# xudoong/EdgeVisionTransformer

Measured on AMD Instinct MI355X. Metric: images/sec DeiT-base/16-224 bs=512 @1/2/4/8 GPU; % bf16 MFMA roofline, higher is better.
Workload: dtype bf16; 1 GPU; deit_base/16-224 forward, bs=512 per GPU, bf16; model=deit_base, global_batch=512, per_gpu_batch=512, seq_len=197, parallelism=dp1, gemm_variant=automatic, lanes=1

## Files before the change

edgevisiontransformer_amd/csrc/attention.hip:

```cpp
#include "common.h"
#include "evt_internal.h"

namespace evt {

namespace {

template <int NKT>
__device__ __forceinline__ float prescale_nonpositive(f32x4 (&s)[NKT], float scale_log2) {
  if (scale_log2 > 0.f) return scale_log2;
#pragma unroll
  for (int kt = 0; kt < NKT; ++kt) s[kt] = s[kt] * scale_log2;
  return 1.f;
}


template <int NKT, bool PLAIN_STORE>
__device__ __forceinline__ void attn_tile_bf16(const AttnParams& p, const EVT_LDS char* Ks,
                                               const EVT_LDS char* Vs, u32x4 qf0, u32x4 qf1,
                                               int qt, int b, int h, int lane) {
  constexpr int ROWB = 128;
  const int g = lane >> 4, c16 = lane & 15, sw = lane & 7;
  f32x4 s[NKT];
#pragma unroll
  for (int kt = 0; kt < NKT; ++kt) {
// ... 155 lines not shown
  }
}

template <int NKT, int WAVES, int NQW, bool NT = false, bool NTQ = NT, bool Q0 = false>
__device__ __forceinline__ void attn_stage_bf16(const AttnParams& p, EVT_LDS char* Ks,
                                                EVT_LDS char* Vs, u32x4 (&qf)[NQW][2], int b,
                                                int h, int wave, int lane) {
  constexpr int NP = NKT * 16, ROWB = 128;
  const bf16* qkv = (const bf16*)p.qkv + b * p.sb + h * p.sh;
  const int g = lane >> 4, c16 = lane & 15;
#pragma unroll
  for (int i = 0; i < NQW; ++i) {
    if (Q0 && wave != 0) break;
    const int qi = min((wave + WAVES * i) * 16 + c16, p.N - 1);
    const bf16* qrow = qkv + (int64_t)qi * p.ldq;
    if (NTQ) {
      qf[i][0] = __builtin_nontemporal_load((const u32x4*)(qrow + 8 * g));
      qf[i][1] = __builtin_nontemporal_load((const u32x4*)(qrow + 8 * (g + 4)));
    } else {
      qf[i][0] = *(const u32x4*)(qrow + 8 * g);
      qf[i][1] = *(const u32x4*)(qrow + 8 * (g + 4));
    }
  }
  const int srow = lane >> 3, sslot = lane & 7;
  for (int i = wave; i < NP / 8; i += WAVES) {
    const int row = i * 8 + srow;
    const int gr = min(row, p.N - 1);
    const bf16* rp = qkv + (int64_t)gr * p.ldq + ((sslot ^ srow) * 8);
    if (NT) {
      __builtin_amdgcn_global_load_lds(rp + p.ko, Ks + i * 8 * ROWB, 16, 0, 2);
// ... 805 lines not shown
  (void)hipFuncSetAttribute((const void*)attn_f32_kernel<14>, hipFuncAttributeMaxDynamicSharedMemorySize,
                      2 * 14 * 16 * 256);
  (void)hipFuncSetAttribute((const void*)attn_f32_kernel<16>, hipFuncAttributeMaxDynamicSharedMemorySize,
                      2 * 16 * 16 * 256);
}

}

bool attention_cls_ok(int dtype, const AttnParams& p) {
  return dtype == DT_BF16 && p.hd == 64 && p.N <= 256 && !p.q8;
}

hipError_t attention_launch(int dtype, const AttnParams& p_in, hipStream_t s) {
  if (p_in.B <= 0) return hipSuccess;
  if (p_in.cls_only && !attention_cls_ok(dtype, p_in)) return hipErrorInvalidValue;
  if (p_in.N <= 0 || p_in.N > EVT_ATTN_MAX_TOKENS || p_in.H <= 0 || p_in.hd <= 0 || p_in.hd > 128)
    return hipErrorInvalidValue;
  if (p_in.N > 256 && p_in.q8) return hipErrorInvalidValue;
  if (p_in.N > 256 && !(p_in.scale_log2 > 0.f && p_in.scale_log2 < INFINITY)) return hipErrorInvalidValue;
  AttnParams p = p_in;
  const bool strided = p.sb || p.sh || p.ko || p.vo;
  if (strided) {
    if (dtype != DT_BF16 || p.hd != 64 || p.q8 || p.sb % 8 || p.sh % 8 || p.ldq % 8 || p.ko % 8 ||
        p.vo % 8 || p.ldq < 64 || p.ko < 0 || p.vo < 0 || p.sb < 0 || p.sh < 0)
      return hipErrorInvalidValue;
  } else {
    p.sb = (int64_t)p.N * p.ldq;
    p.sh = 64;
    p.ko = p.H * 64;
    p.vo = 2 * p.H * 64;
// ... 17 lines not shown
```

edgevisiontransformer_amd/csrc/encoder.cpp:

```cpp
#include "model.h"

using namespace evt;

namespace evt {

int build_encoder(evt_model* m, const float* const* w, hipStream_t s) {
  const int D = m->D;
  const int depth = (int)m->heads.size();
  const int qb = m->standard ? 1 : 0;
  m->layers.resize(depth);
  int k = 0;
  for (int i = 0; i < depth; ++i) {
    Layer& L = m->layers[i];
    L.heads = m->heads[i];
    L.hd = m->head_dim[i];
    L.inner = L.heads * L.hd;
    L.ffn = m->ffn[i];
    L.ffn_st = (int)round_up(L.ffn, PAD_N);
    EVT_RC(copy_vec(m, &L.ln1_g, w[k + 0], D, s));
    EVT_RC(copy_vec(m, &L.ln1_b, w[k + 1], D, s));
    if (m->mx8) {
      EVT_RC(copy_vec(m, &L.ln2_g, w[k + 5], D, s));
      EVT_RC(copy_vec(m, &L.ln2_b, w[k + 6], D, s));
      EVT_RC(make_mx8(m, &L.mqkv, w[k + 2], nullptr, D, 3 * L.inner, s));
// ... 19 lines not shown
void encoder_ws(const Shape& sh, int dtype, bool mx8, int B, size_t hbuf_bytes, WsLayout* l) {
  const size_t es = elem_size(dtype);
  if (dtype == DT_BF16)
    l->bufs.push_back({EVT_WS(sk), gemm_sk_bytes(), 4096, "memset stream-K flags"});
  const size_t rows = (size_t)B * sh.T;
  const size_t xb = (rows * sh.D + PAD_K) * es, ob = (rows * sh.max_inner + PAD_K) * es;
  const size_t stats_bytes = rows * stats_slots(sh.D) * 2 * sizeof(float);
  l->bufs.push_back({EVT_WS(x), xb, xb, "memset x"});
  l->bufs.push_back({EVT_WS(xm), xb, xb, "memset xm"});
  l->bufs.push_back({EVT_WS(sx), stats_bytes});
  l->bufs.push_back({EVT_WS(sm), stats_bytes});
  l->bufs.push_back({EVT_WS(qkv), rows * 3 * sh.max_inner * es});
  l->bufs.push_back({EVT_WS(o), ob, ob, "memset o"});
  l->bufs.push_back({EVT_WS(hbuf), hbuf_bytes});
  l->hbuf_bytes = hbuf_bytes;
  if (!mx8) l->bufs.push_back({EVT_WS(hc), (size_t)B * sh.max_ffn_st * es});
}

int dense_head(const evt_model* m, const DenseW& w, const DenseCall& c, hipStream_t s) {
  const int tiles = ((c.M + GEMM_BM - 1) / GEMM_BM) * (w.npad / GEMM_BN);
  int S = 1;
  while (S < 8 && tiles * S * 2 <= device_cus() && w.kpad % (S * 2 * PAD_K) == 0) S *= 2;
  const size_t part = (size_t)S * std::max(c.M, m->max_batch) * w.npad * sizeof(float);
  if (S < 2 || !m->ws.hbuf || part > m->ws.hbuf_bytes ||
      (c.flags & ~(EPI_BIAS | EPI_GELU | EPI_OUT_F32)))
    return dense(m, w, c, s);
  dense_work(m, w, c);
  const GemmParams p = gemm_operands(c.A, c.lda, w.w, w.kpad, w.npad, c.C, c.ldc, c.M, c.N, w.b,
                                     nullptr, 0, nullptr, 0, 0);
  EVT_HIP(gemm_splitk_launch(m->dtype, c.flags, p, S, (float*)m->ws.hbuf, s), "dense (split-K)");
  return EVT_OK;
}

int run_encoder(evt_model* m, ForwardCall& call) {
  const int B = call.B, D = m->D, T = m->sh.T, rows = B * T;
  hipStream_t s = call.s;
  const float log2e = 1.4426950408889634f;
  m->hm_layers = 0;
  m->tail_mode = 0;
  int block = 0;
  for (const Layer& L : m->layers) {
    const float scale_log2 = log2e / std::sqrt((float)L.hd);
    bool hm = false;
    {
      ProfScope ps(m, EVT_PROF_QKV, s);
      DenseCall c;
      c.flags = EPI_LNIN | EPI_BIAS;
      c.A = m->ws.x; c.lda = D; c.C = m->ws.qkv; c.ldc = 3 * L.inner; c.M = rows; c.N = 3 * L.inner;
      c.stats_in = m->ws.sx;
      if (L.hd == 64 && m->headmajor) {
        DenseCall h = c;
        h.flags |= EPI_HM;
        h.ldc = 64;
        h.P = T;
        if (gemm_headmajor_ok(m->dtype, h.flags, dense_params(m, L.qkv, h))) {
          c = h;
          hm = true;
          ++m->hm_layers;
        }
      }
      EVT_RC(dense(m, L.qkv, c, s));
    }
    AttnParams ap{m->ws.qkv, 3 * L.inner, m->ws.o, L.inner, T, L.heads, B, scale_log2};
    ap.hd = L.hd;
    if (hm) {
      ap.ldq = 64;
      ap.sb = (int64_t)L.heads * 3 * T * 64;
      ap.sh = (int64_t)3 * T * 64;
      ap.ko = T * 64;
      ap.vo = 2 * T * 64;
    }
    const bool last = block + 1 == (int)m->layers.size();
    bool full = !last;
    if (last && call.feat) {
      const evt_features_args* a = call.feat;
      full = a->tokens || (a->n_taps > 0 && a->tap_blocks[a->n_taps - 1] == block);
    }
    if (last) m->tail_mode = full ? 3 : 1;
    {
      ProfScope ps(m, EVT_PROF_ATTENTION, s);
      prof_work(m, 4.0 * B * L.heads * (double)T * T * L.hd,
                (double)rows * 4 * L.inner * elem_size(m->dtype));
      AttnParams aq = ap;
      aq.cls_only = !full && attention_cls_ok(m->dtype, ap);
      EVT_HIP(attention_launch(m->dtype, aq, s), "attention");
    }
    EVT_RC(attn_map(m, call, block, ap));
    EVT_RC(head_stats(m, call, block, ap));
    DenseCall co;
    co.flags = m->standard ? (EPI_BIAS | EPI_RESID | EPI_STATS)
                           : (EPI_BIAS | EPI_RESID | EPI_RESLN | EPI_STATS);
    co.A = m->ws.o; co.lda = L.inner; co.C = m->ws.xm; co.ldc = D; co.M = rows; co.N = D;
    co.resid = m->ws.x; co.ldr = D; co.rstats = m->ws.sx; co.rgamma = L.ln1_g; co.rbeta = L.ln1_b;
    co.stats_out = m->ws.sm;
    DenseCall c1;
    c1.flags = EPI_LNIN | EPI_BIAS | (m->standard ? EPI_GELU_ERF : EPI_GELU);
    c1.A = m->ws.xm; c1.lda = D; c1.C = m->ws.hbuf; c1.ldc = L.ffn_st; c1.M = rows; c1.N = L.ffn_st;
    c1.stats_in = m->ws.sm;
    DenseCall c2;
// ... 79 lines not shown
```

edgevisiontransformer_amd/csrc/evt_internal.h:

```cpp
#pragma once
#include <hip/hip_runtime.h>
#include <stddef.h>
#include <stdint.h>

namespace evt {

enum Dtype : int { DT_F32 = 0, DT_BF16 = 1 };

struct ImgAffine {
  float scale[4], shift[4];
};

enum : int {
  EPI_BIAS = 1,
  EPI_GELU = 2,
  EPI_RESID = 4,
  EPI_POS = 8,
  EPI_OUT_F32 = 16,
  EPI_LNIN = 32,
  EPI_RESLN = 64,
  EPI_STATS = 128,
  EPI_GELU_ERF = 256,
  EPI_OUT_MX8 = 512,
  EPI_GATHER = 1024,
// ... 22 lines not shown
  float eps;
  int nslots;
  int stats_step;
  int rs_step;
  int force_nt;
  int gR, gC;
  float g_inv_rr, g_inv_r;
  int gmode, gOW;
  const void* gzero;
  int* sk_flags;
  float* sk_part;
  int ks_chunk;
  int64_t ks_stride;
  int xgroups;
  int no_balance;
};
constexpr int GEMM_BM = 128;
constexpr int GEMM_BN = 128;
constexpr int PACK_N = 256;
constexpr int PAD_K = 64;
constexpr int PAD_N = 64;

hipError_t gemm_launch(int dtype, int flags, const GemmParams& p, hipStream_t s);
int device_cus();
bool gemm_headmajor_ok(int dtype, int flags, const GemmParams& p);
hipError_t gemm_splitk_launch(int dtype, int flags, const GemmParams& p, int S, float* part,
                              hipStream_t s);
void gemm_set_variant(int v);
size_t gemm_sk_bytes();
void gemm_sk_bind(void* ws, GemmParams& p);
hipError_t pack_weight(int dtype, const float* W, const float* row_scale, int K, int N, void* Wp,
                       int Kpad, int Npad, hipStream_t s);
hipError_t to_bf16_launch(const float* x, void* y, int64_t n, hipStream_t s);
hipError_t ln_fold(int dtype, const void* Wp, int Kpad, const float* W, const float* beta,
                   const float* bias, int K, int N, float* colsum, float* cvec, int Npad,
                   hipStream_t s);

constexpr int EVT_ATTN_MAX_TOKENS = 4096;

struct AttnParams {
  const void* qkv; int64_t ldq;
  void* out;       int64_t ldo;
  int N;
  int H;
  int B;
  float scale_log2;
  uint8_t* q8 = nullptr;
  uint32_t* s8 = nullptr;
  int64_t ldq8 = 0;
  int rows8 = 0;
  int hd = 64;
  int64_t sb = 0, sh = 0;
  int ko = 0, vo = 0;
  int cls_only = 0;
};
hipError_t attention_launch(int dtype, const AttnParams& p, hipStream_t s);
bool attention_cls_ok(int dtype, const AttnParams& p);
hipError_t attn_probs_launch(int dtype, const AttnParams& p, int nq, float* out, hipStream_t s);
hipError_t head_stats_launch(int dtype, const AttnParams& p, int prefix, int grid_w, float* out,
                             hipStream_t s);


hipError_t layernorm_launch(int dtype, const float* x, int64_t ldx, void* y, int64_t ldy,
                            const float* gamma, const float* beta, int rows, int D, float eps,
                            hipStream_t s);

hipError_t export_rows_launch(int dtype, const void* x, int64_t ldx, int64_t row_step, float* out,
                              const float* gamma, const float* beta, int rows, int D, float eps,
                              hipStream_t s);
// ... 121 lines not shown
  ImgAffine aff{};
  const void* w;
  int64_t ldw;
  const float* bias;
  const float* gamma;
  const float* beta;
  void* x;
  float* stats;
  int B, S, nslots;
  float eps;
};
hipError_t swin_embed96_launch(const SwinEmbedParams& p, hipStream_t s);
int gemm_variant();
inline bool gemm_auto() {
  const int v = gemm_variant();
  return v == 0 || v == 30 || v == 31;
}
bool gemm_variant_supported(int v);

struct Mx8GemmParams {
  const uint8_t* A;  int64_t lda;
  const uint32_t* As; int64_t ldas;
  const uint8_t* W;  int64_t ldw;
  const uint32_t* Ws; int64_t ldws;
  void* C;           int64_t ldc;
  uint32_t* Cs;      int64_t ldcs;
  int M, N, K;
  const float* bias;
  const void* resid; int64_t ldr;
  const float* rstats;
  const float* rgamma;
// ... 27 lines not shown
```

edgevisiontransformer_amd/csrc/gemm.hip:

```cpp
#include <type_traits>

#include "common.h"
#include "evt_internal.h"
#include "gemm_epi.h"
#include "gemm_nt.h"
#include "gemm_big8.h"
#include "gemm_big.h"
#include "gemm_pers.h"
#include "gemm_p384.h"
#include "gemm_sk.h"

namespace evt {

namespace {

enum : int {
  V_AUTO = 0,
  V_NT = 1,
  V_BIG_PLAIN = 2,
  V_BIG_SCHED = 6,
  V_BIG8 = 8,
  V_PERS = 9,
  V_STREAMK = 16,
  V_P384 = 30,
  V_NO_P384 = 31,
  V_NO_BALANCE = 36,
};
thread_local int g_gemm_variant = V_AUTO;

int g_num_cus = 0;
const int g_grid_balance = [] {
  const char* e = std::getenv("EVT_GRID_BALANCE");
  return (e && e[0] >= '0' && e[0] <= '2') ? e[0] - '0' : 1;
}();

int num_cus() {
  if (!g_num_cus) {
    int dev = 0;
    hipGetDevice(&dev);
    hipDeviceGetAttribute(&g_num_cus, hipDeviceAttributeMultiprocessorCount, dev);
  }
  return g_num_cus;
// ... 20 lines not shown
         fl == (EPI_BIAS | EPI_RESID | EPI_RESLN | EPI_STATS);
}

constexpr bool p384_fl(int fl) {
  return fl == (EPI_BIAS | EPI_RESID | EPI_RESLN | EPI_STATS) ||
         fl == (EPI_BIAS | EPI_RESID | EPI_STATS) || fl == (EPI_LNIN | EPI_BIAS | EPI_GELU) ||
         fl == (EPI_LNIN | EPI_BIAS);
}

bool use_big(const GemmParams& p, int flags) {
  if (p.force_nt || p.rs_step > 1) return false;
  if ((p.ntiles * GEMM_BN) % BIG_BN) return false;
  if (std::max(std::max(p.lda, p.ldw), std::max(p.ldc, p.resid ? p.ldr : (int64_t)0)) > BIG_MAX_LD)
    return false;
  if (!(flags & EPI_OUT_F32) && p.vec_ok < 2) return false;
  const int v = (g_gemm_variant == V_NO_P384 || g_gemm_variant == V_NO_BALANCE) ? V_AUTO
                                                                                : g_gemm_variant;
  if (v == V_NT) return false;
  if (v != V_AUTO) return true;
  const int64_t G = num_cus();
  const int64_t t256 = (int64_t)((p.M + 255) / 256) * (p.ntiles * GEMM_BN / 256);
  const int64_t t128 = (int64_t)((p.M + 127) / 128) * p.ntiles;
  return (t256 + G - 1) / G <= 0.5 * (double)((t128 + G - 1) / G);
}

bool pers_wide(const GemmParams& p, int flags) {
  return (flags & (EPI_LNIN | EPI_RESLN)) && p.nslots > 8;
}

bool use_pers(const GemmParams& p, int flags) {
  const int v = g_gemm_variant;
  if (v != V_AUTO && v != V_PERS && v != V_STREAMK && v != V_NO_P384 && v != V_NO_BALANCE)
    return false;
  if (p.N % 8 || p.vec_ok < 2 || p.force_nt || p.rs_step > 1) return false;
  if ((flags & (EPI_LNIN | EPI_RESLN)) && (p.nslots > 12 || p.nslots % 2 || p.stats_step > 1))
    return false;
  if (pers_wide(p, flags) &&
      (!pers_wide_fl(flags) || p.K / 64 < PERS_WIDE_MIN_NK || v == V_STREAMK))
    return false;
  if ((flags & EPI_POS) && (!p.resid || p.ldr % 8 || p.P <= 0 || p.M >= (1 << 22))) return false;
  return true;
}

int pers_xgroups(int ntiles, int G, int total) {
  if (G != 256 || total <= G) return 1;
  return (ntiles % 2 == 0 && ntiles / 2 >= 3) ? 2 : 1;
}

bool use_p384(const GemmParams& p, int flags) {
  const int v = g_gemm_variant;
  if ((v != V_AUTO && v != V_P384) || p.N % 384 || p.vec_ok < 2 || p.K < 64) return false;
  if (p.force_nt || p.rs_step > 1) return false;
  if (std::max(std::max(p.lda, p.ldw), std::max(p.ldc, p.resid ? p.ldr : (int64_t)0)) > BIG_MAX_LD)
    return false;
  if ((flags & (EPI_LNIN | EPI_RESLN)) && (p.nslots > 8 || p.nslots % 2 || p.stats_step > 1))
    return false;
  if ((flags & EPI_STATS) && 3 * (p.N / 384) > p.nslots) return false;
  return v == V_P384;
}

constexpr int SK_MAX_G = 256;

int sk_grid() { return min(num_cus(), SK_MAX_G) & ~7; }

bool use_sk(const GemmParams& p) {
  if (!p.sk_flags || !p.sk_part || g_gemm_variant != V_STREAMK) return false;
// ... 17 lines not shown
  if (g_gemm_variant == V_BIG_PLAIN)
    hipLaunchKernelGGL((gemm_big_kernel<FL, 0>), grid, dim3(512), 0, s, q);
  else if (g_gemm_variant == V_BIG8)
    hipLaunchKernelGGL((gemm_big_kernel<FL, 8>), grid, dim3(512), 0, s, q);
  else if constexpr ((FL & EPI_POS) != 0)
    hipLaunchKernelGGL((gemm_big_kernel<FL, 8>), grid, dim3(512), 0, s, q);
  else
    hipLaunchKernelGGL((gemm_big_kernel<FL, 6>), grid, dim3(512), 0, s, q);
  return hipGetLastError();
}

template <int FL>
hipError_t launch_pers(const GemmParams& p, hipStream_t s) {
  num_cus();
  GemmParams q = p;
  q.ntiles = (p.ntiles * GEMM_BN) / BIG_BN;
  const int total = ((p.M + BIG_BM - 1) / BIG_BM) * q.ntiles;
  int G = min(total, g_num_cus);
  if (G >= 8 && total > G) G &= ~7;
  const int rounds = (total + G - 1) / G;
  const int bal = (g_gemm_variant == V_NO_BALANCE || p.no_balance) ? 0 : g_grid_balance;
  if (total > G && G >= 8 && (bal == 2 || (bal == 1 && rounds <= 4)))
    G = min(G, (((total + rounds - 1) / rounds) + 7) & ~7);
  else if (total <= G && (G & 7) && ((G + 7) & ~7) <= max(g_num_cus, 8)) G = (G + 7) & ~7;
  q.xgroups = pers_xgroups(q.ntiles, G, total);
  if constexpr (pers_wide_fl(FL)) {
    if (pers_wide(p, FL)) {
      if (p.N % BIG_BN == 0)
        hipLaunchKernelGGL((gemm_pers_kernel<FL, false, true>), dim3(G), dim3(512), 0, s, q, total);
      else
        hipLaunchKernelGGL((gemm_pers_kernel<FL, true, true>), dim3(G), dim3(512), 0, s, q, total);
// ... 16 lines not shown
  if (G >= 8 && total > G) G &= ~7;
  hipLaunchKernelGGL((gemm_p384_kernel<FL>), dim3(G), dim3(512), 0, s, q, total);
  return hipGetLastError();
}

template <int FL>
hipError_t launch_sk(const GemmParams& p, hipStream_t s) {
  GemmParams q = p;
  q.ntiles = (p.ntiles * GEMM_BN) / BIG_BN;
  const int total = ((p.M + BIG_BM - 1) / BIG_BM) * q.ntiles;
  hipLaunchKernelGGL((gemm_sk_kernel<FL>), dim3(sk_grid()), dim3(512), 0, s, q, total);
  return hipGetLastError();
}

template <typename T, int FL>
hipError_t launch_t(const GemmParams& p, hipStream_t s) {
  if constexpr ((FL & EPI_HM) != 0) {
    if constexpr (std::is_same<T, bf16>::value && pers_fl(FL)) {
      if (headmajor_fits(p) && use_big(p, FL) && use_pers(p, FL)) return launch_pers<FL>(p, s);
    }
    return hipErrorNotSupported;
  } else if constexpr ((FL & (EPI_GATHER | EPI_SPLIT)) != 0) {
    if constexpr (std::is_same<T, bf16>::value) {
      constexpr bool MERGE = (FL & EPI_GATHER) != 0;
      const bool merge = MERGE && p.gmode == 1 && p.gR % 2 == 0 && p.gOW == p.gR / 2 &&
                         p.gC % 8 == 0 && p.K == 4 * p.gC;
      const bool unfold = !MERGE && p.gmode == 2 && p.gC == 64 && p.K == 9 * 64 && p.gzero &&
                          p.gOW == (p.gR + 1) / 2;
      if ((merge || unfold) && p.gR > 0 && p.M < (1 << 22) && use_big(p, FL) && use_pers(p, FL) &&
          !use_sk(p))
        return launch_pers<FL>(p, s);
    }
    return hipErrorNotSupported;
  } else {
    if constexpr (std::is_same<T, bf16>::value) {
      if constexpr (p384_fl(FL)) {
        if (use_p384(p, FL)) return launch_p384<FL>(p, s);
      }
      if (use_big(p, FL)) {
        if constexpr (pers_fl(FL)) {
          if (use_pers(p, FL)) return use_sk(p) ? launch_sk<FL>(p, s) : launch_pers<FL>(p, s);
        }
        return launch_big<FL>(p, s);
      }
    }
    const int mtiles = (p.M + GEMM_BM - 1) / GEMM_BM;
    hipLaunchKernelGGL((gemm_nt_kernel<T, FL>), dim3(mtiles * p.ntiles), dim3(256), 0, s, p);
    return hipGetLastError();
  }
// ... 110 lines not shown
  }
  s = wave_sum(s);
  c = wave_sum(c);
  if (lane == 0) {
    colsum[n] = s;
    cvec[n] = (n < N) ? c + (bias ? bias[n] : 0.f) : 0.f;
  }
}

}

int device_cus() { return num_cus(); }
void gemm_set_variant(int v) { g_gemm_variant = v; }
bool gemm_variant_supported(int v) {
  return v == V_AUTO || v == V_NT || v == V_BIG_PLAIN || v == V_BIG_SCHED || v == V_BIG8 ||
         v == V_PERS || v == V_STREAMK || v == V_P384 || v == V_NO_P384 || v == V_NO_BALANCE;
}
int gemm_variant() { return g_gemm_variant; }

size_t gemm_sk_bytes() { return 4096 + (size_t)SK_MAX_G * SK_SLOT_FLOATS * sizeof(float); }

void gemm_sk_bind(void* ws, GemmParams& p) {
  p.sk_flags = ws ? (int*)ws : nullptr;
  p.sk_part = ws ? (float*)((char*)ws + 4096) : nullptr;
}

bool gemm_headmajor_ok(int dtype, int flags, const GemmParams& p) {
  constexpr int F = EPI_LNIN | EPI_BIAS | EPI_HM;
  return dtype == DT_BF16 && (flags | EPI_HM) == F && p.K % PAD_K == 0 && p.K > 0 &&
         p.ntiles * GEMM_BN >= p.N && headmajor_fits(p) && use_big(p, F) && use_pers(p, F);
}

hipError_t gemm_launch(int dtype, int flags, const GemmParams& p, hipStream_t s) {
  if (p.M <= 0 || p.N <= 0) return hipSuccess;
  if (p.K % PAD_K != 0 || p.K <= 0) return hipErrorInvalidValue;
  if (p.ntiles * GEMM_BN < p.N) return hipErrorInvalidValue;
  return dtype == DT_BF16 ? dispatch<bf16>(flags, p, s) : dispatch<float>(flags, p, s);
}

hipError_t gemm_splitk_launch(int dtype, int flags, const GemmParams& p, int S, float* part,
                              hipStream_t s) {
  if (p.M <= 0 || p.N <= 0) return hipSuccess;
  if (S < 1 || p.K % (S * PAD_K) || (flags & ~(EPI_BIAS | EPI_GELU | EPI_OUT_F32)) || !part)
    return hipErrorInvalidValue;
  return dtype == DT_BF16 ? splitk_t<bf16>(flags, p, S, part, s) : splitk_t<float>(flags, p, S, part, s);
}

namespace {
__global__ void to_bf16_kernel(const float* __restrict__ x, bf16* __restrict__ y, int64_t n) {
  const int64_t i = (int64_t)blockIdx.x * blockDim.x + threadIdx.x;
  if (i < n) y[i] = (bf16)x[i];
// ... 36 lines not shown
```

edgevisiontransformer_amd/csrc/gemm_epi.h:

```cpp
#pragma once
#include <type_traits>

#include "common.h"
#include "evt_internal.h"

namespace evt {

namespace {

constexpr int ROWB = 128;
constexpr int TILE_BYTES = GEMM_BM * ROWB;
constexpr int STAGE_BYTES = 2 * TILE_BYTES;

template <typename T> struct Mma;
template <> struct Mma<bf16> {
  static __device__ __forceinline__ void run(const u32x4& a, const u32x4& b, f32x4& c) {
    c = __builtin_amdgcn_mfma_f32_16x16x32_bf16(__builtin_bit_cast(bf16x8, a),
                                                __builtin_bit_cast(bf16x8, b), c, 0, 0, 0);
  }
};
template <> struct Mma<float> {
  static __device__ __forceinline__ void run(const u32x4& a, const u32x4& b, f32x4& c) {
    const f32x4 af = __builtin_bit_cast(f32x4, a), bf = __builtin_bit_cast(f32x4, b);
#pragma unroll
// ... 16 lines not shown

__device__ __forceinline__ void ln_coef(const float* stats, int nslots, int64_t row, float inv_d,
                                        float eps, float& mu, float& r) {
  const float2* st = (const float2*)(stats + 2 * nslots * row);
  float s1 = 0.f, s2 = 0.f;
  for (int j = 0; j < nslots; ++j) {
    const float2 v = st[j];
    s1 += v.x;
    s2 += v.y;
  }
  mu = s1 * inv_d;
  r = rsqrtf(fmaxf(s2 * inv_d - mu * mu, 0.f) + eps);
}

__device__ __forceinline__ int stg_off(int row, int chunk) { return row * 512 + ((chunk ^ (row & 7)) << 4); }

__device__ __forceinline__ float row_bcast(float v, int l0, int sub) {
  const int a = __builtin_amdgcn_readlane(__builtin_bit_cast(int, v), l0);
  const int b = __builtin_amdgcn_readlane(__builtin_bit_cast(int, v), l0 + 1);
  return __builtin_bit_cast(float, sub ? b : a);
}

template <typename T, int FL, bool INTERIOR>
__device__ __forceinline__ void epi_rows_t(const GemmParams& p, EVT_LDS char* stg, int m0, int n,
                                           int row_lo, int lane, int slot) {
  typedef typename std::conditional<(FL & EPI_OUT_F32) != 0, float, T>::type TO;
  constexpr bool interior = INTERIOR;
  const int sub = lane >> 5, c = lane & 31;
  const bool col_ok = interior || n < p.N;
  const bool full = interior || (p.vec_ok && n + 4 <= p.N);
// ... 16 lines not shown
                p.eps, in_mu, in_r);
      if (FL & EPI_RESLN) ln_coef(p.rstats, p.nslots, (int64_t)mr * rs_step, p.inv_d, p.eps, rs_mu, rs_r);
    }
  }
#pragma unroll
  for (int i = 0; i < 16; ++i) {
    if (i == 8) __builtin_amdgcn_sched_barrier(0);
    const int row = row_lo + 2 * i + sub;
    const int m = m0 + row;
    const bool ok = col_ok && (interior || m < p.M);
    f32x4 v = *(const EVT_LDS f32x4*)(stg + stg_off(row, c));
    int64_t orow = m;
    if (FL & EPI_LNIN) {
      const float mu = row_bcast(in_mu, 2 * i, sub), r = row_bcast(in_r, 2 * i, sub);
      if constexpr (std::is_same<T, float>::value) v = v * r + bias4;
      else v = v * r - cs4 * (r * mu) + bias4;
    } else if (FL & EPI_BIAS) {
      v += bias4;
    }
    if (FL & (EPI_GELU | EPI_GELU_ERF))
      v = gelu4(v, (FL & EPI_GELU) ? 0 : std::is_same<T, bf16>::value ? 2 : 1);
    if (FL & EPI_POS) {
      const int img = m / p.P, t = m - img * p.P;
      orow = (int64_t)img * (p.P + 1) + 1 + t;
      if (ok) v += col4(p.pos + (int64_t)(t + 1) * p.ldp, n, p.N, full);
    }
    if (FL & EPI_RESID) {
      f32x4 rv = f32x4{0.f, 0.f, 0.f, 0.f};
      if (ok) {
        const T* rp = (const T*)p.resid + (int64_t)m * p.ldr + n;
// ... 86 lines not shown
#pragma unroll
  for (int i = 0; i < 8; ++i) {
    if ((FL & EPI_RESID) ? (i & 1) == 0 && i > 0 : i == 4) __builtin_amdgcn_sched_barrier(0);
    const int row = row_lo + 4 * i + q;
    const int m = m0 + row;
    const bool ok = col_ok && (interior || m < p.M);
    const int src = (4 * i + q) * 4;
    f32x4 v[2];
    v[0] = *(const EVT_LDS f32x4*)(stg + stg_off(row, 2 * c8));
    v[1] = *(const EVT_LDS f32x4*)(stg + stg_off(row, 2 * c8 + 1));
    int64_t orow = m;
    if (FL & EPI_LNIN) {
      const float mu = __builtin_bit_cast(float, __builtin_amdgcn_ds_bpermute(src, __builtin_bit_cast(int, in_mu)));
      const float r = __builtin_bit_cast(float, __builtin_amdgcn_ds_bpermute(src, __builtin_bit_cast(int, in_r)));
#pragma unroll
      for (int h = 0; h < 2; ++h) v[h] = v[h] * r - cs4[h] * (r * mu) + bias4[h];
    } else if (FL & EPI_BIAS) {
      v[0] += bias4[0];
      v[1] += bias4[1];
    }
    if (FL & (EPI_GELU | EPI_GELU_ERF)) {
#pragma unroll
      for (int h = 0; h < 2; ++h) v[h] = gelu4(v[h], (FL & EPI_GELU) ? 0 : 2);
    }
    if (FL & EPI_POS) {
      const int img = m / p.P, t = m - img * p.P;
      orow = (int64_t)img * (p.P + 1) + 1 + t;
      if (ok) {
        const float* pr = p.pos + (int64_t)(t + 1) * p.ldp;
        v[0] += col4(pr, n, p.N, interior || n + 4 <= p.N);
        v[1] += col4(pr, n + 4, p.N, full);
// ... 91 lines not shown
```

edgevisiontransformer_amd/csrc/gemm_pers.h:

```cpp
#pragma once
#include "gemm_big8.h"

namespace evt {

namespace {

constexpr int PERS_RAW = 2 * BIG_STAGE;
constexpr int PERS_COLRAW = PERS_RAW + 16384;
constexpr int PERS_COEF = PERS_COLRAW + 3072;
constexpr int PERS_COLB = PERS_COEF + 2048;
constexpr int PERS_PART = PERS_COLB + 3072;
constexpr int PERS_LDS = PERS_PART + 4096;
constexpr int PERS_LDS_ALL = PERS_LDS + 16;
constexpr int PERS_X = 16;
constexpr int PERS_ACC = PERS_LDS_ALL;
constexpr int PERS_LDS_WIDE = PERS_ACC + 2048;
constexpr int PERS_WIDE_MIN_NK = 8;
static_assert(PERS_LDS_WIDE <= 160 * 1024, "LDS of one workgroup");

template <int FL>
struct PersFlags {
  static constexpr bool ln = (FL & (EPI_LNIN | EPI_RESLN)) != 0;
  static constexpr bool v0 = (FL & EPI_BIAS) != 0;
  static constexpr bool v1 = (FL & (EPI_LNIN | EPI_RESLN)) != 0;
// ... 404 lines not shown
template <int FL, bool PADN, typename P = GemmParams, bool WIDE = false>
__device__ __forceinline__ void pers_run(const P& p, int total, int tile, char* smem) {
  constexpr int ER = (FL & EPI_RESID) ? 2 : 0;
  const int tid = threadIdx.x, lane = tid & 63;
  const int wave = __builtin_amdgcn_readfirstlane(tid >> 6);
  const int wm = wave >> 2, wn = wave & 3;
  const int G = gridDim.x;
  const int nk = p.K / 64;
  const int xg = p.xgroups;
  constexpr bool KT2 = (FL & EPI_LNIN) && (FL & (EPI_GELU | EPI_GELU_ERF)) &&
                       !(FL & (EPI_RESID | EPI_HM | EPI_STATS | EPI_GATHER | EPI_SPLIT));
  constexpr bool U2 = !PADN && !(FL & (EPI_GATHER | EPI_SPLIT)) &&
                      !((FL & EPI_RESID) && !(FL & EPI_RESLN));
  int tm, tn;
  pers_tile(tile, G, p.ntiles, xg, total, tm, tn);
  pers_coop_dma<FL, WIDE>(p, smem, wave, lane, tm * BIG_BM, tn * BIG_BN);
  if constexpr (WIDE) {
    wait_vmcnt0();
    big8_bar();
    pers_wide_reduce(smem, tid);
    big8_bar();
    pers_coop_dma<FL, WIDE>(p, smem, wave, lane, tm * BIG_BM, tn * BIG_BN, 1);
  }
  big8_prologue(p, smem, wave, lane, tm * BIG_BM, tn * BIG_BN, nk);
  wait_vmcnt0();
  int par = 0;
  const bool early = nk >= 3;
  while (true) {
    const int m0 = tm * BIG_BM, n0 = tn * BIG_BN;
    f32x4 acc[4][8];
#pragma unroll
    for (int i = 0; i < 4; ++i)
#pragma unroll
      for (int j = 0; j < 8; ++j) acc[i][j] = f32x4{0.f, 0.f, 0.f, 0.f};
    int ln = lane;
    asm volatile("" : "+v"(ln));
    u32x4 rre[2][4];
    const int next = tile + G;
    int ntm = 0, ntn = 0;
    const bool has_next = pers_tile(next, G, p.ntiles, xg, total, ntm, ntn);
    if (!has_next) ntm = ntn = 0;
    const bool cont = has_next && nk >= 2;
    const int npar = cont ? par ^ (nk & 1) : 0;
    auto last = [&]() {
      if constexpr (ER > 0) pers_resid_early<0, 1>(p, wm, wn, ln, m0, n0, rre);
    };
    auto last3 = [&]() {
      if constexpr (ER > 1) pers_resid_early<1, 2>(p, wm, wn, ln, m0, n0, rre);
    };
    if (early) {
      auto pre1 = [&]() { pers_coef<FL, WIDE>(p, smem, tid - 256); };
      auto mid = [&]() {
        if (has_next) pers_coop_dma<FL, WIDE>(p, smem, wave, lane, ntm * BIG_BM, ntn * BIG_BN);
      };
      auto after = [&](int t) {
// ... 66 lines not shown
```

edgevisiontransformer_amd/csrc/model.cpp:

```cpp
#include "model.h"

using namespace evt;

namespace evt {

static thread_local std::string g_err;

int fail(int code, const std::string& msg) {
  g_err = msg;
  return code;
}

int hip_fail(hipError_t e, const char* what) {
  return fail(EVT_EHIP, std::string(what) + ": " + hipGetErrorString(e));
}

bool qkv_headmajor_default() {
  const char* e = std::getenv("EVT_QKV_LAYOUT");
  return !(e && std::strcmp(e, "token") == 0);
}

void prof_reset(evt_model* m) {
  if (!m->prof) return;
  m->prof_role.clear();
// ... 136 lines not shown
                               c.resid, c.ldr, c.pos, c.ldp, c.P);
  p.colsum = w.colsum;
  p.no_balance = m->no_balance;
  p.stats_in = c.stats_in;
  p.rstats = c.rstats;
  p.rgamma = c.rgamma;
  p.rbeta = c.rbeta;
  p.stats_out = c.stats_out;
  const int width = c.ln_width ? c.ln_width : m->D;
  p.inv_d = 1.0f / (float)width;
  p.eps = m->eps;
  p.nslots = stats_slots(c.slot_width ? c.slot_width : width);
  p.stats_step = c.stats_step;
  p.rs_step = c.rs_step;
  p.force_nt = c.force_nt;
  gemm_sk_bind(m->ws.sk, p);
  return p;
}

int dense(const evt_model* m, const DenseW& w, const DenseCall& c, hipStream_t s) {
  dense_work(m, w, c);
  const GemmParams p = dense_params(m, w, c);
  EVT_HIP(gemm_launch(m->dtype, c.flags, p, s), "dense");
  return EVT_OK;
}

int feat_export(evt_model* m, const void* x, int64_t ldx, int64_t row_step, float* out, bool norm,
                int rows, int D, hipStream_t s) {
  ProfScope ps(m, EVT_PROF_HEAD, s);
  prof_work(m, 0.0, (double)rows * D * (elem_size(m->dtype) + 4.0));
// ... 629 lines not shown
```

edgevisiontransformer_amd/csrc/model.h:

```cpp
#pragma once
#include <hip/hip_runtime.h>

#include <algorithm>
#include <cmath>
#include <cstddef>
#include <cstdio>
#include <cstdlib>
#include <cstring>
#include <functional>
#include <string>
#include <type_traits>
#include <vector>

#include "../../include/evt.h"
#include "evt_internal.h"

#pragma GCC visibility push(hidden)

namespace evt {

int fail(int code, const std::string& msg);
int hip_fail(hipError_t e, const char* what);

#define EVT_HIP(call, what)                            \
// ... 223 lines not shown
  int64_t ldr = 0;
  const float* pos = nullptr;
  int64_t ldp = 0;
  int P = 0;
  const float* stats_in = nullptr;
  const float* rstats = nullptr;
  const float* rgamma = nullptr;
  const float* rbeta = nullptr;
  float* stats_out = nullptr;
  int ln_width = 0;
  int stats_step = 1;
  int slot_width = 0;
  int rs_step = 1;
  bool force_nt = false;
  int work_M = 0;
};

struct WsBuf {
  size_t member;
  size_t bytes;
  size_t zeroed = 0;
  const char* what = nullptr;
};
struct WsLayout {
  std::vector<WsBuf> bufs;
  size_t hbuf_bytes = 0;
  int qa_ld = 0, qh_ld = 0;
  bool patch_in_hbuf = false;
  size_t bytes() const {
    size_t n = 0;
// ... 80 lines not shown
```

edgevisiontransformer_amd/csrc/ops.cpp:

```cpp
#include "model.h"

using namespace evt;

int evt::validate_classify(const evt_classify_args* a, int B, int C, int64_t ldl,
                           ClassifyParams* p) {
  if (!a) return fail(EVT_EINVAL, "classify: the classify arguments are NULL");
  if (B < 1) return fail(EVT_EINVAL, "classify: batch must be at least 1");
  if (C < 1 || C > (1 << 20)) return fail(EVT_EINVAL, "classify: num_classes must be in [1, 2^20]");
  if (ldl < C) return fail(EVT_EINVAL, "classify: ldl must be at least num_classes");
  const int kmax = std::min(C, EVT_CLASSIFY_MAX_K);
  if (a->k < 1 || a->k > kmax)
    return fail(EVT_EINVAL, "classify: k must be in [1, min(num_classes, EVT_CLASSIFY_MAX_K) = " +
                                std::to_string(kmax) + "]");
  if (a->values != EVT_CLASSIFY_PROB && a->values != EVT_CLASSIFY_LOGIT)
    return fail(EVT_EINVAL, "classify: values must be EVT_CLASSIFY_PROB or EVT_CLASSIFY_LOGIT");
  if (!a->indices && !a->vals && !a->lse && !a->rank && !a->counters)
    return fail(EVT_EINVAL, "classify: no output requested: indices, vals, lse, rank and counters "
                            "are NULL");
  if ((a->rank || a->counters) && !a->labels)
    return fail(EVT_EINVAL, "classify: rank and counters need labels");
  if (((uintptr_t)a->indices | (uintptr_t)a->vals | (uintptr_t)a->lse | (uintptr_t)a->labels |
       (uintptr_t)a->rank) & 3)
    return fail(EVT_EINVAL, "classify: indices, vals, lse, labels and rank must be 4-byte aligned");
  if ((uintptr_t)a->counters & 7)
    return fail(EVT_EINVAL, "classify: counters must be 8-byte aligned");
  p->k = a->k;
  p->values = a->values == EVT_CLASSIFY_LOGIT ? CLS_LOGIT : CLS_PROB;
  p->indices = a->indices; p->vals = a->vals; p->lse = a->lse;
  p->labels = a->labels; p->rank = a->rank; p->counters = (long long*)a->counters;
  return EVT_OK;
}

extern "C" {

int evt_set_gemm_variant(int variant) {
  if (!gemm_variant_supported(variant))
    return fail(EVT_EINVAL, "variant must be 0, 1, 2, 6, 8, 9, 16, 30, 31 or 36");
  gemm_set_variant(variant);
  return EVT_OK;
}

int evt_pack_weight(int dtype, const float* W, const float* row_scale, int K, int N, void* Wp,
                    int Kpad, int Npad, void* stream) {
  if (!W || !Wp || K <= 0 || N <= 0 || Kpad < K || Npad < N || Kpad % PAD_K || Npad % GEMM_BN)
    return fail(EVT_EINVAL, "pack: bad shape (Npad % 128, Kpad % 64, Kpad >= K, Npad >= N)");
  EVT_HIP(pack_weight(dtype, W, row_scale, K, N, Wp, Kpad, Npad, (hipStream_t)stream),
          "pack_weight");
  return EVT_OK;
}

int evt_mx8_quantize(int in_dtype, const void* x, int64_t ldx, int rows, int K, int Kpad, void* q,
                     int64_t ldq, uint32_t* scales, int64_t ld_s, void* stream) {
// ... 454 lines not shown
```

Measured before the change: 31220 images/s.

## Compute only CLS query rows in last block's QKV projection

In the last encoder block, when only the CLS output is needed, the QKV GEMM is split. The K and V columns are computed for all tokens through a column-window launch. The Q columns are computed only for the CLS row of each image into a small side buffer, and the CLS-only attention reads its query from that buffer. This removes about a third of the last block's QKV GEMM work, at the cost of an extra small launch, new tile-window plumbing in the persistent GEMM, and an FMA-form LN epilogue meant to match the full-path numerics.

Measured after the change: 31300 images/s (median of 6 runs). About the same (+0.2%).

```diff
diff --git a/edgevisiontransformer_amd/csrc/attention.hip b/edgevisiontransformer_amd/csrc/attention.hip
--- a/edgevisiontransformer_amd/csrc/attention.hip
+++ b/edgevisiontransformer_amd/csrc/attention.hip
@@ -193,6 +193,7 @@
     if (Q0 && wave != 0) break;
     const int qi = min((wave + WAVES * i) * 16 + c16, p.N - 1);
     const bf16* qrow = qkv + (int64_t)qi * p.ldq;
+    if (Q0 && p.qcls) qrow = (const bf16*)p.qcls + b * p.ldqcls + h * 64;
     if (NTQ) {
       qf[i][0] = __builtin_nontemporal_load((const u32x4*)(qrow + 8 * g));
       qf[i][1] = __builtin_nontemporal_load((const u32x4*)(qrow + 8 * (g + 4)));
@@ -1028,6 +1029,9 @@
 hipError_t attention_launch(int dtype, const AttnParams& p_in, hipStream_t s) {
   if (p_in.B <= 0) return hipSuccess;
   if (p_in.cls_only && !attention_cls_ok(dtype, p_in)) return hipErrorInvalidValue;
+  if (p_in.qcls && (!p_in.cls_only || p_in.ldqcls < (int64_t)p_in.H * 64 || p_in.ldqcls % 8 ||
+                    ((uintptr_t)p_in.qcls & 15)))
+    return hipErrorInvalidValue;
   if (p_in.N <= 0 || p_in.N > EVT_ATTN_MAX_TOKENS || p_in.H <= 0 || p_in.hd <= 0 || p_in.hd > 128)
     return hipErrorInvalidValue;
   if (p_in.N > 256 && p_in.q8) return hipErrorInvalidValue;
diff --git a/edgevisiontransformer_amd/csrc/encoder.cpp b/edgevisiontransformer_amd/csrc/encoder.cpp
--- a/edgevisiontransformer_amd/csrc/encoder.cpp
+++ b/edgevisiontransformer_amd/csrc/encoder.cpp
@@ -57,7 +57,8 @@
   l->bufs.push_back({EVT_WS(o), ob, ob, "memset o"});
   l->bufs.push_back({EVT_WS(hbuf), hbuf_bytes});
   l->hbuf_bytes = hbuf_bytes;
-  if (!mx8) l->bufs.push_back({EVT_WS(hc), (size_t)B * sh.max_ffn_st * es});
+  if (!mx8)
+    l->bufs.push_back({EVT_WS(hc), (size_t)B * std::max(sh.max_ffn_st, sh.max_inner) * es});
 }
 
 int dense_head(const evt_model* m, const DenseW& w, const DenseCall& c, hipStream_t s) {
@@ -84,6 +85,22 @@
   int block = 0;
   for (const Layer& L : m->layers) {
     const float scale_log2 = log2e / std::sqrt((float)L.hd);
+    const bool last = block + 1 == (int)m->layers.size();
+    bool full = !last;
+    if (last && call.feat) {
+      const evt_features_args* a = call.feat;
+      full = a->tokens || (a->n_taps > 0 && a->tap_blocks[a->n_taps - 1] == block);
+    }
+    if (last) m->tail_mode = full ? 3 : 1;
+    AttnParams ap{m->ws.qkv, 3 * L.inner, m->ws.o, L.inner, T, L.heads, B, scale_log2};
+    ap.hd = L.hd;
+    const bool wants_q =
+        window_attn_wanted(call, block) ||
+        (call.hstats && call.hstats_next < call.hstats->n_blocks &&
+         call.hstats->blocks[call.hstats_next] == block);
+    const int kv0 = L.inner / PACK_N;
+    const bool kv_only = !full && attention_cls_ok(m->dtype, ap) && !wants_q && kv0 > 0 &&
+                         m->ws.hc && gemm_variant() != 37;
     bool hm = false;
     {
       ProfScope ps(m, EVT_PROF_QKV, s);
@@ -102,10 +119,23 @@
           ++m->hm_layers;
         }
       }
-      EVT_RC(dense(m, L.qkv, c, s));
-    }
-    AttnParams ap{m->ws.qkv, 3 * L.inner, m->ws.o, L.inner, T, L.heads, B, scale_log2};
-    ap.hd = L.hd;
+      if (kv_only) {
+        DenseCall q = c;
+        q.flags = EPI_LNIN | EPI_BIAS;
+        q.lda = (int64_t)D * T; q.C = m->ws.hc; q.ldc = L.inner; q.M = B; q.N = L.inner; q.P = 0;
+        q.stats_step = T;
+        q.force_nt = true;
+        q.work_M = -1;
+        q.tnn = (L.inner + PACK_N - 1) / PACK_N;
+        q.lnin_fma = gemm_lnin_fma_form(m->dtype, c.flags, dense_params(m, L.qkv, c));
+        c.tn0 = kv0;
+        c.tnn = L.qkv.npad / PACK_N - kv0;
+        EVT_RC(dense(m, L.qkv, c, s));
+        EVT_RC(dense(m, L.qkv, q, s));
+      } else {
+        EVT_RC(dense(m, L.qkv, c, s));
+      }
+    }
     if (hm) {
       ap.ldq = 64;
       ap.sb = (int64_t)L.heads * 3 * T * 64;
@@ -113,19 +143,16 @@
       ap.ko = T * 64;
       ap.vo = 2 * T * 64;
     }
-    const bool last = block + 1 == (int)m->layers.size();
-    bool full = !last;
-    if (last && call.feat) {
-      const evt_features_args* a = call.feat;
-      full = a->tokens || (a->n_taps > 0 && a->tap_blocks[a->n_taps - 1] == block);
-    }
-    if (last) m->tail_mode = full ? 3 : 1;
     {
       ProfScope ps(m, EVT_PROF_ATTENTION, s);
       prof_work(m, 4.0 * B * L.heads * (double)T * T * L.hd,
                 (double)rows * 4 * L.inner * elem_size(m->dtype));
       AttnParams aq = ap;
       aq.cls_only = !full && attention_cls_ok(m->dtype, ap);
+      if (kv_only) {
+        aq.qcls = m->ws.hc;
+        aq.ldqcls = L.inner;
+      }
       EVT_HIP(attention_launch(m->dtype, aq, s), "attention");
     }
     EVT_RC(attn_map(m, call, block, ap));
diff --git a/edgevisiontransformer_amd/csrc/evt_internal.h b/edgevisiontransformer_amd/csrc/evt_internal.h
--- a/edgevisiontransformer_amd/csrc/evt_internal.h
+++ b/edgevisiontransformer_amd/csrc/evt_internal.h
@@ -60,6 +60,8 @@
   int64_t ks_stride;
   int xgroups;
   int no_balance;
+  int lnin_fma;
+  int tn0, tnn;
 };
 constexpr int GEMM_BM = 128;
 constexpr int GEMM_BN = 128;
@@ -70,6 +72,7 @@
 hipError_t gemm_launch(int dtype, int flags, const GemmParams& p, hipStream_t s);
 int device_cus();
 bool gemm_headmajor_ok(int dtype, int flags, const GemmParams& p);
+bool gemm_lnin_fma_form(int dtype, int flags, const GemmParams& p);
 hipError_t gemm_splitk_launch(int dtype, int flags, const GemmParams& p, int S, float* part,
                               hipStream_t s);
 void gemm_set_variant(int v);
@@ -99,6 +102,8 @@
   int64_t sb = 0, sh = 0;
   int ko = 0, vo = 0;
   int cls_only = 0;
+  const void* qcls = nullptr;
+  int64_t ldqcls = 0;
 };
 hipError_t attention_launch(int dtype, const AttnParams& p, hipStream_t s);
 bool attention_cls_ok(int dtype, const AttnParams& p);
@@ -250,7 +255,7 @@
 int gemm_variant();
 inline bool gemm_auto() {
   const int v = gemm_variant();
-  return v == 0 || v == 30 || v == 31;
+  return v == 0 || v == 30 || v == 31 || v == 37;
 }
 bool gemm_variant_supported(int v);
 
diff --git a/edgevisiontransformer_amd/csrc/gemm.hip b/edgevisiontransformer_amd/csrc/gemm.hip
--- a/edgevisiontransformer_amd/csrc/gemm.hip
+++ b/edgevisiontransformer_amd/csrc/gemm.hip
@@ -25,7 +25,9 @@
   V_P384 = 30,
   V_NO_P384 = 31,
   V_NO_BALANCE = 36,
+  V_FULL_QKV = 37,
 };
+bool variant_auto(int v) { return v == V_AUTO || v == V_FULL_QKV; }
 thread_local int g_gemm_variant = V_AUTO;
 
 int g_num_cus = 0;
@@ -76,8 +78,10 @@
   if (std::max(std::max(p.lda, p.ldw), std::max(p.ldc, p.resid ? p.ldr : (int64_t)0)) > BIG_MAX_LD)
     return false;
   if (!(flags & EPI_OUT_F32) && p.vec_ok < 2) return false;
-  const int v = (g_gemm_variant == V_NO_P384 || g_gemm_variant == V_NO_BALANCE) ? V_AUTO
-                                                                                : g_gemm_variant;
+  const int v = (g_gemm_variant == V_NO_P384 || g_gemm_variant == V_NO_BALANCE ||
+                 g_gemm_variant == V_FULL_QKV)
+                    ? V_AUTO
+                    : g_gemm_variant;
   if (v == V_NT) return false;
   if (v != V_AUTO) return true;
   const int64_t G = num_cus();
@@ -92,7 +96,7 @@
 
 bool use_pers(const GemmParams& p, int flags) {
   const int v = g_gemm_variant;
-  if (v != V_AUTO && v != V_PERS && v != V_STREAMK && v != V_NO_P384 && v != V_NO_BALANCE)
+  if (!variant_auto(v) && v != V_PERS && v != V_STREAMK && v != V_NO_P384 && v != V_NO_BALANCE)
     return false;
   if (p.N % 8 || p.vec_ok < 2 || p.force_nt || p.rs_step > 1) return false;
   if ((flags & (EPI_LNIN | EPI_RESLN)) && (p.nslots > 12 || p.nslots % 2 || p.stats_step > 1))
@@ -111,7 +115,7 @@
 
 bool use_p384(const GemmParams& p, int flags) {
   const int v = g_gemm_variant;
-  if ((v != V_AUTO && v != V_P384) || p.N % 384 || p.vec_ok < 2 || p.K < 64) return false;
+  if ((!variant_auto(v) && v != V_P384) || p.N % 384 || p.vec_ok < 2 || p.K < 64) return false;
   if (p.force_nt || p.rs_step > 1) return false;
   if (std::max(std::max(p.lda, p.ldw), std::max(p.ldc, p.resid ? p.ldr : (int64_t)0)) > BIG_MAX_LD)
     return false;
@@ -159,7 +163,7 @@
 hipError_t launch_pers(const GemmParams& p, hipStream_t s) {
   num_cus();
   GemmParams q = p;
-  q.ntiles = (p.ntiles * GEMM_BN) / BIG_BN;
+  q.ntiles = p.tnn ? p.tnn : (p.ntiles * GEMM_BN) / BIG_BN;
   const int total = ((p.M + BIG_BM - 1) / BIG_BM) * q.ntiles;
   int G = min(total, g_num_cus);
   if (G >= 8 && total > G) G &= ~7;
@@ -206,6 +210,30 @@
 }
 
 template <typename T, int FL>
+hipError_t launch_window(const GemmParams& p, hipStream_t s) {
+  if constexpr ((FL & (EPI_STATS | EPI_POS | EPI_RESID | EPI_OUT_F32)) != 0) {
+    return hipErrorNotSupported;
+  } else {
+    if constexpr (std::is_same<T, bf16>::value && pers_fl(FL)) {
+      if (use_big(p, FL) && use_pers(p, FL) && !use_sk(p)) return launch_pers<FL>(p, s);
+    }
+    const int c0 = p.tn0 * BIG_BN;
+    if (c0 >= p.N) return hipSuccess;
+    GemmParams q = p;
+    q.W = (const T*)p.W + (int64_t)c0 * p.ldw;
+    q.C = (T*)p.C + c0;
+    if (p.bias) q.bias = p.bias + c0;
+    if (p.colsum) q.colsum = p.colsum + c0;
+    q.N = min(p.N - c0, p.tnn * BIG_BN);
+    q.ntiles = (q.N + GEMM_BN - 1) / GEMM_BN;
+    q.tn0 = q.tnn = 0;
+    const int mtiles = (p.M + GEMM_BM - 1) / GEMM_BM;
+    hipLaunchKernelGGL((gemm_nt_kernel<T, FL>), dim3(mtiles * q.ntiles), dim3(256), 0, s, q);
+    return hipGetLastError();
+  }
+}
+
+template <typename T, int FL>
 hipError_t launch_t(const GemmParams& p, hipStream_t s) {
   if constexpr ((FL & EPI_HM) != 0) {
     if constexpr (std::is_same<T, bf16>::value && pers_fl(FL)) {
@@ -225,6 +253,7 @@
     }
     return hipErrorNotSupported;
   } else {
+    if (p.tnn) return launch_window<T, FL>(p, s);
     if constexpr (std::is_same<T, bf16>::value) {
       if constexpr (p384_fl(FL)) {
         if (use_p384(p, FL)) return launch_p384<FL>(p, s);
@@ -365,7 +394,8 @@
 void gemm_set_variant(int v) { g_gemm_variant = v; }
 bool gemm_variant_supported(int v) {
   return v == V_AUTO || v == V_NT || v == V_BIG_PLAIN || v == V_BIG_SCHED || v == V_BIG8 ||
-         v == V_PERS || v == V_STREAMK || v == V_P384 || v == V_NO_P384 || v == V_NO_BALANCE;
+         v == V_PERS || v == V_STREAMK || v == V_P384 || v == V_NO_P384 || v == V_NO_BALANCE ||
+         v == V_FULL_QKV;
 }
 int gemm_variant() { return g_gemm_variant; }
 
@@ -382,10 +412,20 @@
          p.ntiles * GEMM_BN >= p.N && headmajor_fits(p) && use_big(p, F) && use_pers(p, F);
 }
 
+bool gemm_lnin_fma_form(int dtype, int flags, const GemmParams& p) {
+  constexpr int F = EPI_LNIN | EPI_BIAS;
+  if (dtype != DT_BF16 || (flags & ~EPI_HM) != F) return false;
+  if (flags & EPI_HM) return true;
+  return use_p384(p, F) || (use_big(p, F) && use_pers(p, F));
+}
+
 hipError_t gemm_launch(int dtype, int flags, const GemmParams& p, hipStream_t s) {
   if (p.M <= 0 || p.N <= 0) return hipSuccess;
   if (p.K % PAD_K != 0 || p.K <= 0) return hipErrorInvalidValue;
   if (p.ntiles * GEMM_BN < p.N) return hipErrorInvalidValue;
+  if (p.tnn && (p.tn0 < 0 || p.tnn < 0 || (p.tn0 + p.tnn) * (BIG_BN / GEMM_BN) > p.ntiles ||
+                (flags & (EPI_GATHER | EPI_SPLIT))))
+    return hipErrorInvalidValue;
   return dtype == DT_BF16 ? dispatch<bf16>(flags, p, s) : dispatch<float>(flags, p, s);
 }
 
diff --git a/edgevisiontransformer_amd/csrc/gemm_epi.h b/edgevisiontransformer_amd/csrc/gemm_epi.h
--- a/edgevisiontransformer_amd/csrc/gemm_epi.h
+++ b/edgevisiontransformer_amd/csrc/gemm_epi.h
@@ -54,6 +54,13 @@
 }
 
 __device__ __forceinline__ int stg_off(int row, int chunk) { return row * 512 + ((chunk ^ (row & 7)) << 4); }
+
+__device__ __forceinline__ f32x4 lnin_fma4(f32x4 acc, f32x4 cs, float mu, float r, f32x4 c) {
+  f32x4 o;
+#pragma unroll
+  for (int j = 0; j < 4; ++j) o[j] = __builtin_fmaf(__builtin_fmaf(cs[j], -mu, acc[j]), r, c[j]);
+  return o;
+}
 
 __device__ __forceinline__ float row_bcast(float v, int l0, int sub) {
   const int a = __builtin_amdgcn_readlane(__builtin_bit_cast(int, v), l0);
@@ -100,6 +107,7 @@
     if (FL & EPI_LNIN) {
       const float mu = row_bcast(in_mu, 2 * i, sub), r = row_bcast(in_r, 2 * i, sub);
       if constexpr (std::is_same<T, float>::value) v = v * r + bias4;
+      else if (p.lnin_fma) v = lnin_fma4(v, cs4, mu, r, bias4);
       else v = v * r - cs4 * (r * mu) + bias4;
     } else if (FL & EPI_BIAS) {
       v += bias4;
@@ -216,7 +224,9 @@
       const float mu = __builtin_bit_cast(float, __builtin_amdgcn_ds_bpermute(src, __builtin_bit_cast(int, in_mu)));
       const float r = __builtin_bit_cast(float, __builtin_amdgcn_ds_bpermute(src, __builtin_bit_cast(int, in_r)));
 #pragma unroll
-      for (int h = 0; h < 2; ++h) v[h] = v[h] * r - cs4[h] * (r * mu) + bias4[h];
+      for (int h = 0; h < 2; ++h)
+        v[h] = p.lnin_fma ? lnin_fma4(v[h], cs4[h], mu, r, bias4[h])
+                          : v[h] * r - cs4[h] * (r * mu) + bias4[h];
     } else if (FL & EPI_BIAS) {
       v[0] += bias4[0];
       v[1] += bias4[1];
diff --git a/edgevisiontransformer_amd/csrc/gemm_pers.h b/edgevisiontransformer_amd/csrc/gemm_pers.h
--- a/edgevisiontransformer_amd/csrc/gemm_pers.h
+++ b/edgevisiontransformer_amd/csrc/gemm_pers.h
@@ -442,6 +442,7 @@
                       !((FL & EPI_RESID) && !(FL & EPI_RESLN));
   int tm, tn;
   pers_tile(tile, G, p.ntiles, xg, total, tm, tn);
+  tn += p.tn0;
   pers_coop_dma<FL, WIDE>(p, smem, wave, lane, tm * BIG_BM, tn * BIG_BN);
   if constexpr (WIDE) {
     wait_vmcnt0();
@@ -467,6 +468,7 @@
     const int next = tile + G;
     int ntm = 0, ntn = 0;
     const bool has_next = pers_tile(next, G, p.ntiles, xg, total, ntm, ntn);
+    ntn += p.tn0;
     if (!has_next) ntm = ntn = 0;
     const bool cont = has_next && nk >= 2;
     const int npar = cont ? par ^ (nk & 1) : 0;
diff --git a/edgevisiontransformer_amd/csrc/model.cpp b/edgevisiontransformer_amd/csrc/model.cpp
--- a/edgevisiontransformer_amd/csrc/model.cpp
+++ b/edgevisiontransformer_amd/csrc/model.cpp
@@ -174,6 +174,9 @@
   p.stats_step = c.stats_step;
   p.rs_step = c.rs_step;
   p.force_nt = c.force_nt;
+  p.lnin_fma = c.lnin_fma;
+  p.tn0 = c.tn0;
+  p.tnn = c.tnn;
   gemm_sk_bind(m->ws.sk, p);
   return p;
 }
diff --git a/edgevisiontransformer_amd/csrc/model.h b/edgevisiontransformer_amd/csrc/model.h
--- a/edgevisiontransformer_amd/csrc/model.h
+++ b/edgevisiontransformer_amd/csrc/model.h
@@ -261,6 +261,8 @@
   int rs_step = 1;
   bool force_nt = false;
   int work_M = 0;
+  int tn0 = 0, tnn = 0;
+  bool lnin_fma = false;
 };
 
 struct WsBuf {
diff --git a/edgevisiontransformer_amd/csrc/ops.cpp b/edgevisiontransformer_amd/csrc/ops.cpp
--- a/edgevisiontransformer_amd/csrc/ops.cpp
+++ b/edgevisiontransformer_amd/csrc/ops.cpp
@@ -35,7 +35,8 @@
 
 int evt_set_gemm_variant(int variant) {
   if (!gemm_variant_supported(variant))
-    return fail(EVT_EINVAL, "variant must be 0, 1, 2, 6, 8, 9, 16, 30, 31 or 36");
+    return fail(EVT_EINVAL, "variant must be 0, 1, 2, 6, 8, 9, 16, 30, 31 or 36 (kernel selection), or 37 (the last "
+                "encoder block's full QKV launch)");
   gemm_set_variant(variant);
   return EVT_OK;
 }
```
